# NOAA-GFDL/pace

Hardware: AMD Instinct MI355X
Metric: simulated-days/day + acoustic-step ms, C768 L79 fp64, 1/2/4/8 MI355X (higher is better)
Workload: dtype f64

## Files before the change

pace_amd/build.py:

```python
from __future__ import annotations

import argparse
import concurrent.futures as cf
import hashlib
import os
import subprocess
import sys

HERE = os.path.dirname(os.path.abspath(__file__))
CSRC = os.path.join(HERE, "csrc")
ROOT = os.path.dirname(HERE)
HOSTEMU_DIR = os.path.join(ROOT, "tests", "_hostemu")

SOURCES = ["fv3_ctx.hip", "fv3_tp2d.hip", "fv3_tp2x.hip", "fv3_tp4.hip", "fv3_tp4x.hip", "fv3_a2b.hip", "fv3_csw.hip", "fv3_dsw.hip", "fv3_wind.hip", "fv3_nh.hip", "fv3_del2x.hip", "fv3_pgf.hip", "fv3_step.hip", "fv3_halo.hip", "fv3_tracer.hip", "fv3_remap.hip", "fv3_c2l.hip", "fv3_diag.hip"]
HEADERS = ["fv3_common.h", "fv3_ops.h", "fv3_ppm.h", "fv3_a2b.h", "fv3_math.h", "fv3_agpr.h", "fv3_march.h", os.path.join("..", "..", "include", "fv3_mi355x.h")]

HIPCC = os.environ.get("HIPCC", "/opt/rocm/bin/hipcc")
HIP_FLAGS = ["--offload-arch=gfx950", "-std=c++17", "-O3", "-ffp-contract=off", "-fPIC", "-fno-gpu-rdc", "-Wno-unused-result"]
HOST_FLAGS = ["-x", "c++", "-std=c++17", "-O2", "-ffp-contract=off", "-fopenmp", "-fPIC", "-DFV3_HOST_EMU"]


def _tag() -> str:
    t = os.environ.get("FV3_LIB_TAG", "")
    return ("." + t) if t else ""


def lib_path(precision: int = 64, hostemu: bool = False) -> str:
    if hostemu:
        return os.path.join(HOSTEMU_DIR, f"libfv3_hostemu_f{precision}.so")
    return os.path.join(CSRC, f"libfv3_mi355x_f{precision}{_tag()}.so")


def _digest(paths, extra):
    h = hashlib.sha256()
    for p in paths:
        with open(p, "rb") as f:
            h.update(f.read())
    h.update(repr(extra).encode())
    return h.hexdigest()


def src_hash() -> str:
    paths = [os.path.join(CSRC, s) for s in SOURCES] + [os.path.normpath(os.path.join(CSRC, h)) for h in HEADERS]
    return _digest(paths, None)[:16]


def variant_suffix() -> str:
    extra = os.environ.get("FV3_EXTRA_FLAGS", "").split()
    per = sorted((k, v) for k, v in os.environ.items() if k.startswith("FV3_FLAGS_") and v.strip())
    tag = os.environ.get("FV3_LIB_TAG", "")
    if not extra and not per and not tag:
        return ""
    return "+" + hashlib.sha256(repr((extra, per)).encode()).hexdigest()[:8] + (("." + tag) if tag else "")


def _run(cmd):
    r = subprocess.run(cmd, capture_output=True, text=True)
    if r.returncode != 0:
        raise RuntimeError("build failed: " + " ".join(cmd) + "\n" + r.stdout + r.stderr)


def build(precision: int = 64, hostemu: bool = False, force: bool = False, verbose: bool = True) -> str:
    out = lib_path(precision, hostemu)
    objdir = os.path.join(HOSTEMU_DIR if hostemu else CSRC, f"_obj_f{precision}{'' if hostemu else _tag()}")
    os.makedirs(objdir, exist_ok=True)
    srcs = [os.path.join(CSRC, s) for s in SOURCES]
    hdrs = [os.path.normpath(os.path.join(CSRC, h)) for h in HEADERS]
    real = [] if precision == 64 else ["-DFV3_REAL=float"]
# ... 48 lines not shown
```

pace_amd/csrc/fv3_a2b.h:

```cpp
#pragma once
#include "fv3_ops.h"

#define A2B_A1 ((Real)0.5625)
#define A2B_A2 ((Real)-0.0625)
#define A2B_B1 ((Real)(7.0 / 12.0))
#define A2B_B2 ((Real)(-1.0 / 12.0))
#define A2B_C1 ((Real)(2.0 / 3.0))
#define A2B_C2 ((Real)(-1.0 / 6.0))
#define A2B_R3 ((Real)(1.0 / 3.0))

namespace {

struct A2B {
  const Geo &g;
  const Real *q;
  MPtr dxa;
  MPtr dya;
  bool W, E, S, N;

  Real sc;
  FV3_HD Real Q(int i, int j) const { return sc * q[IX(i, j)]; }

  FV3_HD Real qx_int(int i, int j) const { return A2B_B2 * (Q(i - 2, j) + Q(i + 1, j)) + A2B_B1 * (Q(i - 1, j) + Q(i, j)); }
  FV3_HD Real qy_int(int i, int j) const { return A2B_B2 * (Q(i, j - 2) + Q(i, j + 1)) + A2B_B1 * (Q(i, j - 1) + Q(i, j)); }

  FV3_HD Real qx_w1(int j) const {
    const Real g_in = dxa[IX(2, j)] / dxa[IX(1, j)], g_ou = dxa[IX(-1, j)] / dxa[IX(0, j)];
    return (Real)0.5 * ((((Real)2 + g_in) * Q(1, j) - Q(2, j)) / ((Real)1 + g_in) + (((Real)2 + g_ou) * Q(0, j) - Q(-1, j)) / ((Real)1 + g_ou));
  }
  FV3_HD Real qx_e1(int j) const {
    const int npx = g.npx;
    const Real g_in = dxa[IX(npx - 2, j)] / dxa[IX(npx - 1, j)], g_ou = dxa[IX(npx + 1, j)] / dxa[IX(npx, j)];
    return (Real)0.5 *
           ((((Real)2 + g_in) * Q(npx - 1, j) - Q(npx - 2, j)) / ((Real)1 + g_in) + (((Real)2 + g_ou) * Q(npx, j) - Q(npx + 1, j)) / ((Real)1 + g_ou));
  }
  FV3_HD Real qx(int i, int j) const {
    const int npx = g.npx;
    if (W) {
      if (i == 1) return qx_w1(j);
      if (i == 2) {
        const Real g_in = dxa[IX(2, j)] / dxa[IX(1, j)];
        return ((Real)3 * (g_in * Q(1, j) + Q(2, j)) - (g_in * qx_w1(j) + qx_int(3, j))) / ((Real)2 + (Real)2 * g_in);
      }
    }
    if (E) {
      if (i == npx) return qx_e1(j);
      if (i == npx - 1) {
        const Real g_in = dxa[IX(npx - 2, j)] / dxa[IX(npx - 1, j)];
        return ((Real)3 * (Q(npx - 2, j) + g_in * Q(npx - 1, j)) - (g_in * qx_e1(j) + qx_int(npx - 2, j))) / ((Real)2 + (Real)2 * g_in);
      }
    }
    return qx_int(i, j);
  }
  FV3_HD Real qy_s1(int i) const {
    const Real g_in = dya[IX(i, 2)] / dya[IX(i, 1)], g_ou = dya[IX(i, -1)] / dya[IX(i, 0)];
    return (Real)0.5 * ((((Real)2 + g_in) * Q(i, 1) - Q(i, 2)) / ((Real)1 + g_in) + (((Real)2 + g_ou) * Q(i, 0) - Q(i, -1)) / ((Real)1 + g_ou));
  }
  FV3_HD Real qy_n1(int i) const {
    const int npy = g.npy;
    const Real g_in = dya[IX(i, npy - 2)] / dya[IX(i, npy - 1)], g_ou = dya[IX(i, npy + 1)] / dya[IX(i, npy)];
    return (Real)0.5 *
           ((((Real)2 + g_in) * Q(i, npy - 1) - Q(i, npy - 2)) / ((Real)1 + g_in) + (((Real)2 + g_ou) * Q(i, npy) - Q(i, npy + 1)) / ((Real)1 + g_ou));
  }
  FV3_HD Real qy(int i, int j) const {
    const int npy = g.npy;
    if (S) {
      if (j == 1) return qy_s1(i);
      if (j == 2) {
        const Real g_in = dya[IX(i, 2)] / dya[IX(i, 1)];
        return ((Real)3 * (g_in * Q(i, 1) + Q(i, 2)) - (g_in * qy_s1(i) + qy_int(i, 3))) / ((Real)2 + (Real)2 * g_in);
      }
    }
    if (N) {
      if (j == npy) return qy_n1(i);
      if (j == npy - 1) {
        const Real g_in = dya[IX(i, npy - 2)] / dya[IX(i, npy - 1)];
        return ((Real)3 * (Q(i, npy - 2) + g_in * Q(i, npy - 1)) - (g_in * qy_n1(i) + qy_int(i, npy - 2))) / ((Real)2 + (Real)2 * g_in);
      }
    }
    return qy_int(i, j);
  }
  FV3_HD Real q2x(int ie_, int j) const {
    return (Q(ie_ - 1, j) * dxa[IX(ie_, j)] + Q(ie_, j) * dxa[IX(ie_ - 1, j)]) / (dxa[IX(ie_ - 1, j)] + dxa[IX(ie_, j)]);
  }
  FV3_HD Real q1y(int i, int je_) const {
    return (Q(i, je_ - 1) * dya[IX(i, je_)] + Q(i, je_) * dya[IX(i, je_ - 1)]) / (dya[IX(i, je_ - 1)] + dya[IX(i, je_)]);
  }
  FV3_HD Real edge_x(int ie_, int j, Real w) const { return w * q2x(ie_, j - 1) + ((Real)1 - w) * q2x(ie_, j); }
  FV3_HD Real edge_y(int i, int je_, Real w) const { return w * q1y(i - 1, je_) + ((Real)1 - w) * q1y(i, je_); }
  FV3_HD Real qxx_int(int i, int j) const { return A2B_A2 * (qx(i, j - 2) + qx(i, j + 1)) + A2B_A1 * (qx(i, j - 1) + qx(i, j)); }
  FV3_HD Real qyy_int(int i, int j) const { return A2B_A2 * (qy(i - 2, j) + qy(i + 1, j)) + A2B_A1 * (qy(i - 1, j) + qy(i, j)); }
};

FV3_HD inline Real extrap(Real fac, Real q1, Real q2) { return q1 + fac * (q1 - q2); }

FV3_HD inline __attribute__((always_inline)) Real a2b_point(const Geo &g, const Real *qlev, int t, int i, int j, Real scale = (Real)1) {
  const int fl = g.flags[t];
  const A2B a{g, qlev, g.dxa + t * g.st2, g.dya + t * g.st2, (fl & FV3_W) != 0, (fl & FV3_E) != 0, (fl & FV3_S) != 0, (fl & FV3_N) != 0, scale};
  const int npx = g.npx, npy = g.npy;
  const bool onW = a.W && i == 1, onE = a.E && i == npx, onS = a.S && j == 1, onN = a.N && j == npy;
  const Real *ce = g.corner_extrap + t * 12;
  Real r;
  if ((!a.W || i >= 3) && (!a.E || i <= npx - 2) && (!a.S || j >= 3) && (!a.N || j <= npy - 2)) {
    const Real *q = a.q;
    Real qx[4], qy[4];
#pragma unroll
    for (int n = 0; n < 4; ++n) {
      const int jj = j - 2 + n, ii = i - 2 + n;
      qx[n] = A2B_B2 * (scale * q[IX(i - 2, jj)] + scale * q[IX(i + 1, jj)]) + A2B_B1 * (scale * q[IX(i - 1, jj)] + scale * q[IX(i, jj)]);
      qy[n] = A2B_B2 * (scale * q[IX(ii, j - 2)] + scale * q[IX(ii, j + 1)]) + A2B_B1 * (scale * q[IX(ii, j - 1)] + scale * q[IX(ii, j)]);
    }
    const Real qxx = A2B_A2 * (qx[0] + qx[3]) + A2B_A1 * (qx[1] + qx[2]);
    const Real qyy = A2B_A2 * (qy[0] + qy[3]) + A2B_A1 * (qy[1] + qy[2]);
    r = (Real)0.5 * (qxx + qyy);
  } else if (onW && onS) {
    r = (extrap(ce[0], a.Q(1, 1), a.Q(2, 2)) + extrap(ce[1], a.Q(0, 1), a.Q(-1, 2)) + extrap(ce[2], a.Q(1, 0), a.Q(2, -1))) * A2B_R3;
  } else if (onE && onS) {
    r = (extrap(ce[3], a.Q(npx - 1, 1), a.Q(npx - 2, 2)) + extrap(ce[4], a.Q(npx - 1, 0), a.Q(npx - 2, -1)) + extrap(ce[5], a.Q(npx, 1), a.Q(npx + 1, 2))) *
        A2B_R3;
  } else if (onE && onN) {
    r = (extrap(ce[6], a.Q(npx - 1, npy - 1), a.Q(npx - 2, npy - 2)) + extrap(ce[7], a.Q(npx, npy - 1), a.Q(npx + 1, npy - 2)) +
         extrap(ce[8], a.Q(npx - 1, npy), a.Q(npx - 2, npy + 1))) *
        A2B_R3;
  } else if (onW && onN) {
    r = (extrap(ce[9], a.Q(1, npy - 1), a.Q(2, npy - 2)) + extrap(ce[10], a.Q(0, npy - 1), a.Q(-1, npy - 2)) + extrap(ce[11], a.Q(1, npy), a.Q(2, npy + 1))) *
        A2B_R3;
  } else if (onW) {
    r = a.edge_x(1, j, g.edge_w[t * g.nj + j + g.o]);
  } else if (onE) {
    r = a.edge_x(npx, j, g.edge_e[t * g.nj + j + g.o]);
  } else if (onS) {
    r = a.edge_y(i, 1, g.edge_s[t * g.ni + i + g.o]);
  } else if (onN) {
    r = a.edge_y(i, npy, g.edge_n[t * g.ni + i + g.o]);
  } else {
    Real qxx, qyy;
    if (a.S && j == 2)
      qxx = A2B_C1 * (a.qx(i, 1) + a.qx(i, 2)) + A2B_C2 * (a.edge_y(i, 1, g.edge_s[t * g.ni + i + g.o]) + a.qxx_int(i, 3));
    else if (a.N && j == npy - 1)
      qxx = A2B_C1 * (a.qx(i, npy - 2) + a.qx(i, npy - 1)) + A2B_C2 * (a.edge_y(i, npy, g.edge_n[t * g.ni + i + g.o]) + a.qxx_int(i, npy - 2));
    else
      qxx = a.qxx_int(i, j);
    if (a.W && i == 2)
      qyy = A2B_C1 * (a.qy(1, j) + a.qy(2, j)) + A2B_C2 * (a.edge_x(1, j, g.edge_w[t * g.nj + j + g.o]) + a.qyy_int(3, j));
    else if (a.E && i == npx - 1)
      qyy = A2B_C1 * (a.qy(npx - 2, j) + a.qy(npx - 1, j)) + A2B_C2 * (a.edge_x(npx, j, g.edge_e[t * g.nj + j + g.o]) + a.qyy_int(npx - 2, j));
    else
      qyy = a.qyy_int(i, j);
    r = (Real)0.5 * (qxx + qyy);
  }
  return r;
}

}

#define AB_OUT 61
#define AB_PF 4

struct A2bStore {
  Real *out;
  long st, sk;
  FV3_HD void operator()(int t, int k, unsigned p, Real v) const { (out + t * st + k * sk)[p] = v; }
};
template <int WPE, class Epi>
static void a2b_ord4_t(fv3_ctx *c, fv3_stream_t s, const Real *qin, int kin0, int kout0, int nk, Real scale, Epi epi) {
  const Geo g = c->g;
  const int kshift = kout0 - kin0;
  const Geo *gp = c->g_dev;
  const int nx = g.nx, ny = g.ny, nh = g.nh, npx = g.npx, npy = g.npy, sj32 = g.sj32, go = g.o;
  const long st = g.st, sk = g.sk;
  const int nstrip = (nx + 1 + AB_OUT - 1) / AB_OUT;
  const int seg = fv3_pick_seg((long)nstrip * ((ny + 64) / 64) * g.nsub * nk, 8);
  int nseg = (ny + 1 + seg / 2) / seg;
  if (nseg < 1) nseg = 1;
  const int seglen = (ny + 1 + nseg - 1) / nseg;
  const size_t smem = sizeof(Real) * 2 * (FV3_WAVE + 3);
  launch_waves<WPE>(c, s, nstrip, nseg, g.nsub * nk, smem, [=] FV3_HD(const Blk &blk, char *smem_) {
    const int t = blk.bz / nk, k = kin0 + (blk.bz - t * nk);
    const int fl = gp->flags[t];
    const Real *q = qin + t * st + k * sk;
    const int ia = (fl & FV3_W) ? 3 : 1, ib = (fl & FV3_E) ? npx - 2 : nx + 1;
    const int ja = (fl & FV3_S) ? 3 : 1, jb = (fl & FV3_N) ? npy - 2 : ny + 1;
    const int i0 = 1 + blk.bx * AB_OUT;
    int j0 = 1 + blk.by * seglen, j1 = j0 + seglen - 1;
    if (j0 < ja) j0 = ja;
    if (j1 > jb) j1 = jb;
    if (j0 > j1) return;
    const int ilo = i0 > ia ? i0 : ia, ihi = i0 + AB_OUT - 1 < ib ? i0 + AB_OUT - 1 : ib;
    if (ilo > ihi) return;
    Real *lq = (Real *)smem_ + 2;
    Real *ly = lq + FV3_WAVE + 3;
    const int ied = nx + nh;
    Real qa[FV3_LPT], qb[FV3_LPT], qc[FV3_LPT], qd[FV3_LPT];
    Real x0[FV3_LPT], x1[FV3_LPT], x2[FV3_LPT], x3[FV3_LPT];
    Real pf[AB_PF][FV3_LPT];
    unsigned pcol[FV3_LPT];
    bool own[FV3_LPT];
    const int r_beg = j0 - 2, r_end = j1 + 1;
    FV3_LANES(blk, lane, l) {
      const int i = i0 - 2 + lane, ic = i < ied ? i : ied;
      pcol[l] = (unsigned)(go * sj32 + ic + go);
      own[l] = i >= ilo && i <= ihi;
      qa[l] = qb[l] = qc[l] = qd[l] = x0[l] = x1[l] = x2[l] = x3[l] = (Real)0;
      if (lane < 2) lq[lane - 2] = ly[lane - 2] = (Real)0;
      if (lane == 0) lq[FV3_WAVE] = ly[FV3_WAVE] = (Real)0;
// ... 57 lines not shown
```

pace_amd/csrc/fv3_dsw.hip:

```cpp
#include "fv3_a2b.h"
#include "fv3_ops.h"
#include "fv3_ppm.h"

namespace {

struct FxAdv {
  Geo g;
  const Real *uc, *vc;
  long m2;
  Real dt;
  bool W, E, S, N;

  FV3_HD Real UC(int i, int j) const { return uc[IX(i, j)]; }
  FV3_HD Real VC(int i, int j) const { return vc[IX(i, j)]; }
  FV3_HD Real ut_gen(int i, int j) const {
    return (UC(i, j) - (Real)0.25 * (g.cosa_u + m2)[IX(i, j)] * (VC(i - 1, j) + VC(i, j) + VC(i - 1, j + 1) + VC(i, j + 1))) * (g.rsin_u + m2)[IX(i, j)];
  }
  FV3_HD Real vt_gen(int i, int j) const {
    return (VC(i, j) - (Real)0.25 * (g.cosa_v + m2)[IX(i, j)] * (UC(i, j - 1) + UC(i + 1, j - 1) + UC(i, j) + UC(i + 1, j))) * (g.rsin_v + m2)[IX(i, j)];
  }
  FV3_HD bool edge_col(int i) const { return (W && i == 1) || (E && i == g.npx); }
  FV3_HD bool edge_row(int j) const { return (S && j == 1) || (N && j == g.npy); }
  FV3_HD bool ut_special_row(int j) const { return (S && (j == 0 || j == 1)) || (N && (j == g.npy - 1 || j == g.npy)); }
  FV3_HD Real ut_edge(int i, int j) const {
// ... 775 lines not shown
  } else {
    for (int w = 0; w < wins.n; ++w) {
      Wins one, pone;
      one.n = pone.n = 1;
      one.w[0] = wins.w[w];
      pone.w[0] = patches.w[w];
      run(one, pone, &needs[w]);
    }
  }
}

bool dsw_honors_acc_first(const fv3_ctx *c) {
  int nmax = 0;
  for (int k = 0; k < c->g.nz; ++k) nmax = std::max(nmax, std::max(c->nord_v_h[k], std::max(c->nord_w_h[k], c->nord_t_h[k])));
  const char *sc_env = getenv("FV3_DSW_SCALARS");
  return !(sc_env && !strcmp(sc_env, "separate")) && nmax <= 2 && c->zeros;
}

struct AccSlots {
  const Real *crx[FV3_ACC_MAXSTEPS], *cry[FV3_ACC_MAXSTEPS];
};
static int acc_sum(fv3_ctx *c, Real *cx, Real *cy, int n, void *stream) {
  if (n < 1 || n > FV3_ACC_MAXSTEPS || (int)c->acc_slots.size() < 2 * n) return fv3_fail(c, FV3_ERR_ARG, "acc_sum: no Courant-number slots for this many sub-steps");
  AccSlots sl;
  for (int q = 0; q < FV3_ACC_MAXSTEPS; ++q) {
    const int m = q < n ? q : n - 1;
    sl.crx[q] = c->acc_slots[2 * m];
    sl.cry[q] = c->acc_slots[2 * m + 1];
  }
  const Geo g = c->g;
  const int isd = 1 - g.nh, ied = g.nx + g.nh, jsd = 1 - g.nh, jed = g.ny + g.nh;
  launch3<4>(c, (fv3_stream_t)stream, Box{isd, ied, jsd, jed, 0, g.nz - 1}, [=] FV3_HD(int t, int k, int i, int j) {
    const long p = t * g.st + k * g.sk + IX(i, j);
    if (i >= 1 && i <= g.nx + 1) {
      Real a = (Real)0 + sl.crx[0][p];
#pragma unroll
      for (int q = 1; q < FV3_ACC_MAXSTEPS; ++q)
        if (q < n) a = a + sl.crx[q][p];
      cx[p] = a;
    }
    if (j >= 1 && j <= g.ny + 1) {
      Real a = (Real)0 + sl.cry[0][p];
#pragma unroll
      for (int q = 1; q < FV3_ACC_MAXSTEPS; ++q)
        if (q < n) a = a + sl.cry[q][p];
      cy[p] = a;
    }
  });
  return fv3_post(c, (fv3_stream_t)stream, "acc_sum");
}

bool dsw_can_defer_acc(const fv3_ctx *c) { return dsw_honors_acc_first(c); }

int fv3_d_sw_out(fv3_ctx *c, const fv3_field *delpc_, const fv3_field *delp_, const fv3_field *pt_, const fv3_field *u_, const fv3_field *v_,
                 const fv3_field *w_, const fv3_field *uc_, const fv3_field *vc_, const fv3_field *ua_, const fv3_field *va_,
                 const fv3_field *divgd_, const fv3_field *mfx_, const fv3_field *mfy_, const fv3_field *cx_, const fv3_field *cy_,
                 const fv3_field *crx_, const fv3_field *cry_, const fv3_field *xfx_, const fv3_field *yfx_, const fv3_field *q_con_,
                 const fv3_field *zh_, const fv3_field *heat_source_, const fv3_field *diss_est_, double dtd, void *stream,
                 const fv3_field *o_delp_, const fv3_field *o_pt_, const fv3_field *o_w_, const fv3_field *o_q_con_, int (*after_scalars)(void *), void *after_user) {
  if (!c) return FV3_ERR_ARG;
  FV3_FIELD(delpc, delpc_) FV3_FIELD(delp, delp_) FV3_FIELD(pt, pt_) FV3_FIELD(u, u_) FV3_FIELD(v, v_) FV3_FIELD(w, w_) FV3_FIELD(uc, uc_)
  FV3_FIELD(vc, vc_) FV3_FIELD(ua, ua_) FV3_FIELD(va, va_) FV3_FIELD(divgd, divgd_) FV3_FIELD(mfx, mfx_) FV3_FIELD(mfy, mfy_) FV3_FIELD(cx, cx_)
  FV3_FIELD(cy, cy_) FV3_FIELD(crx, crx_) FV3_FIELD(cry, cry_) FV3_FIELD(xfx, xfx_) FV3_FIELD(yfx, yfx_) FV3_FIELD(q_con, q_con_)
  FV3_FIELD(heat_source, heat_source_)
  (void)zh_;
  (void)diss_est_;
  const bool oop = o_delp_ != nullptr;
  Real *o_delp = delp, *o_pt = pt, *o_w = w, *o_q_con = q_con;
  if (oop) {
    if (!o_pt_ || !o_w_ || !o_q_con_) return fv3_fail(c, FV3_ERR_ARG, "d_sw: the four output fields come together");
    o_delp = fv3_chk(c, o_delp_, "o_delp");
    o_pt = fv3_chk(c, o_pt_, "o_pt");
    o_w = fv3_chk(c, o_w_, "o_w");
    o_q_con = fv3_chk(c, o_q_con_, "o_q_con");
    if (!o_delp || !o_pt || !o_w || !o_q_con) return FV3_ERR_ARG;
    if (o_delp == delp || o_pt == pt || o_w == w || o_q_con == q_con) return fv3_fail(c, FV3_ERR_ARG, "d_sw: an output field aliases its input");
  }
  const Geo g = c->g;
  fv3_stream_t s = (fv3_stream_t)stream;
  const Real dt = (Real)dtd;
  const fv3_acoustic_config cf = c->cfg;
  const DampTables tab = c->tab;
  const int nz1 = g.nz - 1;
  const int isd = 1 - g.nh, ied = g.nx + g.nh, jsd = 1 - g.nh, jed = g.ny + g.nh;
  Real *ut = c->scratch[SC_A], *vt = c->scratch[SC_B], *fx = c->scratch[SC_C], *fy = c->scratch[SC_D], *gx = c->scratch[SC_E], *gy = c->scratch[SC_F];
  Real *heat_s = c->scratch[SC_H], *ke = c->scratch[SC_I], *wk = c->scratch[SC_J];
  int nord_max_v = 0, nord_max_w = 0, nord_max_t = 0, nord_max = 0;
  for (int k = 0; k < g.nz; ++k) {
    nord_max_v = std::max(nord_max_v, c->nord_v_h[k]);
    nord_max_w = std::max(nord_max_w, c->nord_w_h[k]);
    nord_max_t = std::max(nord_max_t, c->nord_t_h[k]);
    nord_max = std::max(nord_max, c->nord_h[k]);
  }

  fv3_stream_t s2 = fv3_aux(c, s);
  Real *dA_x = c->scratch[SC_DN_FX], *dA_y = c->scratch[SC_DN_FY], *dB_x = c->scratch[SC_S], *dB_y = c->scratch[SC_T], *d2w = c->scratch[SC_DN_D2];
  Deln dn_vt{g.nord_v, tab.tp_vt, g.damp_vt, 0, (Real)0, false, (Real)1.0e-4, nord_max_v};
  Deln dn_w{g.nord_w, tab.d6_w, g.damp_w, 0, (Real)0, false, (Real)1.0e-5, nord_max_w};
  Deln dn_t{g.nord_t, tab.tp_t, g.damp_t, 0, (Real)0, false, (Real)1.0e-4, nord_max_t};
  const char *sc_env = getenv("FV3_DSW_SCALARS");
  const bool fused_scalars = !(sc_env && !strcmp(sc_env, "separate")) && nord_max_v <= 2 && nord_max_t <= 2 && nord_max_w <= 2;
  if (c->seq_acc_first && !fused_scalars) return fv3_fail(c, FV3_ERR_ARG, "d_sw: the sequencer's first-sub-step form of the accumulators needs the fused scalar marches");
  const int scalars_mode = sc_env && !strcmp(sc_env, "quad") ? 0 : 1;
  const bool acc_defer = c->seq_acc_defer;
  if (acc_defer && !fused_scalars) return fv3_fail(c, FV3_ERR_ARG, "d_sw: the sequencer's deferred accumulation needs the fused scalar marches (fxadv with the Courant numbers)");
  if (fused_scalars) {
// ... 294 lines not shown
    const Real vd = damp * d;
    (vdamp + b)[p] = vd;
    (ke + b)[p] += vd;
  });
  Real *dnew = divgd;
  {
    if (!dd_sep) {
      divdamp_staged(c, s, divgd, uc, vc, nord_max, 0, nz1, nullptr);
    } else if (nord_max > 0) {
      dnew = c->scratch[SC_L];
      if (ks1 >= 0) divdamp_stream(c, ss, divgd, dnew, uc, vc, c->scratch[SC_M], nord_max, 0, ks1);
    }
  }
  {
    const Real dddmp = (Real)cf.dddmp;
    const bool keep_divgd = !(c->seq_divgd_dead && dd_sep);
    if (ks1 >= 0) a2b_ord4_t<8>(c, ss, wk, 0, 0, ks1 + 1, (Real)1, [=] FV3_HD(int t, int k, unsigned p, Real wkbv) {
      const int nord = g.nord[k];
      if (nord == 0) return;
      const long b = t * g.st + k * g.sk;
      const Real dpc = dd_sep ? (divgd + b)[p] : (delpc + b)[p];
      Real vo = (Real)0;
      if (dddmp >= (Real)1.0e-5) vo = fabs(dt) * sqrt(dpc * dpc + wkbv * wkbv);
      const Real damp2 = g.da_min_c * fv3_max(g.d2_divg[k], fv3_min((Real)0.20, dddmp * vo));
      const Real dn_ = (dnew + b)[p];
      if (keep_divgd) (divgd + b)[p] = dn_;
      const Real vd = damp2 * dpc + tab.dd8[k] * dn_;
      (vdamp + b)[p] = vd;
      (ke + b)[p] += vd;
    });
    if (ss != s) fv3_signal(c, ss, 4);
    if (kfz <= nz1) {
      Real *const wuc = c->scratch[SC_TP_FY2], *const wvc = c->scratch[SC_TP_FX2];
      dd_copy_windows(c, s, uc, vc, wuc, wvc, kfz, nz1, 2);
      divdamp_patches(c, s, divgd, dnew, wuc, wvc, c->scratch[SC_M], nord_max, kfz, nz1);
      WindStage ws{u, v, uc, vc, divgd, ke, vdamp, wk, dnew, tab.dd8, dt, dddmp, cf.hord_mt, keep_divgd, kfz, nz1};
      const char *sd = getenv("FV3_DSW_SIDE");
      if (heat_in_march && s == s_main && !(sd && !strcmp(sd, "copy"))) {
        ws.u_side = c->scratch[SC_N];
        ws.v_side = c->scratch[SC_O];
        ws.side_seg = sx_march_seg(c, nz1 - fdw_k0 + 1);
        side_from = kfz;
      }
      if (getenv("FV3_DEBUG_FD")) fprintf(stderr, "[d_sw] side copies by the wind stage: %s (segment %d)\n", ws.u_side ? "yes" : "no", ws.side_seg);
      wind_stage_march(c, s, ws);
      launch_frame_w(c, s, Frame{{Box{1, 3, 1, g.ny + 1, kfz, nz1}, Box{g.npx - 2, g.npx, 1, g.ny + 1, 0, 0}, Box{1, g.nx + 1, 1, 3, 0, 0}, Box{1, g.nx + 1, g.npy - 2, g.npy, 0, 0}}},
                     [=] FV3_HD(int w_, int t, int k, int i, int j) {
        const int fl = g.flags[t];
        if (!(fl & (w_ == 0 ? FV3_W : w_ == 1 ? FV3_E : w_ == 2 ? FV3_S : FV3_N))) return;
        if (w_ >= 2 && (((fl & FV3_W) && i <= 3) || ((fl & FV3_E) && i >= g.npx - 2))) return;
        ke_point(t, k, i, j);
      });
      const int nfr = g.nx + 1 > g.ny + 1 ? g.nx + 1 : g.ny + 1;
      launch3(c, s, Box{1, nfr, 1, 12, kfz, nz1}, [=] FV3_HD(int t, int k, int a_, int side) {
        const int fl = g.flags[t];
        int i, j;
        if (side <= 6) {
          if (a_ > g.ny + 1) return;
          if (!(fl & (side <= 3 ? FV3_W : FV3_E))) return;
          i = side <= 3 ? side : g.npx - 6 + side;
          j = a_;
        } else {
          if (a_ > g.nx + 1) return;
          if (!(fl & (side <= 9 ? FV3_S : FV3_N))) return;
          j = side <= 9 ? side - 6 : g.npy - 12 + side;
          i = a_;
          if (((fl & FV3_W) && i <= 3) || ((fl & FV3_E) && i >= g.npx - 2)) return;
        }
        const long b = t * g.st + k * g.sk;
        const unsigned p = IX(i, j);
        const Real wkbv = a2b_point(g, wk + b, t, i, j);
        const Real dpc = (divgd + b)[p];
        Real vo = (Real)0;
        if (dddmp >= (Real)1.0e-5) vo = fabs(dt) * sqrt(dpc * dpc + wkbv * wkbv);
        const Real damp2 = g.da_min_c * fv3_max(g.d2_divg[k], fv3_min((Real)0.20, dddmp * vo));
        const Real vd = damp2 * dpc + tab.dd8[k] * (dnew + b)[p];
        (vdamp + b)[p] = vd;
        (ke + b)[p] += vd;
      });
      dd_copy_windows(c, s, wuc, wvc, uc, vc, kfz, nz1, 0);
      if (keep_divgd) launch3(c, s, Box{1, g.nx + 1, 1, g.ny + 1, kfz, nz1}, [=] FV3_HD(int t, int k, int i, int j) {
        const long pp = t * g.st + k * g.sk + IX(i, j);
        divgd[pp] = dnew[pp];
      });
    }
  }

  };
  static const bool wind_overlap_off = !(getenv("FV3_DSW_WIND_OVERLAP") && getenv("FV3_DSW_WIND_OVERLAP")[0] == '1');
  for (int k = 0; k < g.nz; ++k) keep_uv_dx = keep_uv_dx || (c->d_con_h[k] > 1.0e-5 && !(c->damp_vt_h[k] > 1.0e-5));
  const bool wind_overlap = fused_scalars && s2 != s && !wind_overlap_off && !keep_uv_dx;
  if (wind_overlap) {
    fv3_wait(c, s2, 5);
    wind_branch(s2);
    fv3_signal(c, s2, 6);
  }

  if (after_scalars) {
    const int hst = after_scalars(after_user);
    if (hst != FV3_OK) return hst;
  }
  if (wind_overlap)
    fv3_wait(c, s, 6);
  else
    wind_branch(s);
  if (sponge_forked) fv3_wait(c, s, 4);

// ... 75 lines not shown
```

pace_amd/csrc/fv3_pgf.hip:

```cpp
#include "fv3_a2b.h"
#include "fv3_math.h"

#ifndef PG_WPE
#define PG_WPE (sizeof(Real) == 4 ? 3 : 2)
#endif

namespace {

#define PG_OUT 60
#define PG_PF 2
#define PG_NF 7
#ifndef PG_KB
#define PG_KB 16
#endif

struct PgfArgs {
  const Real *pp, *pk3, *gz, *delp;
  Real *u, *v;
  Real dt, top, gz_scale;
  int nz;
};

struct PgfCorner {
  Real g0, g1, k0, k1, q0, q1, w;
};

FV3_HD inline void pgf_update(const Geo &g, const PgfArgs &a, int t, int k, int i, int j, unsigned p, const PgfCorner &c, const PgfCorner &e, const PgfCorner &n, Real rx,
                              Real ry) {
  const long b = t * g.st + k * g.sk;
  const Real wkp = c.k1 - c.k0;
  if (i <= g.nx) {
    const Real du = a.dt / (wkp + (e.k1 - e.k0)) * ((c.g1 - e.g0) * (e.k1 - c.k0) + (c.g0 - e.g1) * (c.k1 - e.k0));
    (a.u + b)[p] = ((a.u + b)[p] + du + a.dt / (c.w + e.w) * ((c.g1 - e.g0) * (e.q1 - c.q0) + (c.g0 - e.g1) * (c.q1 - e.q0))) * rx;
  }
  if (j <= g.ny) {
    const Real dv = a.dt / (wkp + (n.k1 - n.k0)) * ((c.g1 - n.g0) * (n.k1 - c.k0) + (c.g0 - n.g1) * (c.k1 - n.k0));
    (a.v + b)[p] = ((a.v + b)[p] + dv + a.dt / (c.w + n.w) * ((c.g1 - n.g0) * (n.q1 - c.q0) + (c.g0 - n.g1) * (c.q1 - n.q0))) * ry;
  }
}

FV3_HD inline void pgf_march_range(const Geo &g, int fl, int &ia, int &ib, int &ja, int &jb) {
  ia = (fl & FV3_W) ? 3 : 1;
  ib = (fl & FV3_E) ? g.npx - 3 : g.nx + 1;
  ja = (fl & FV3_S) ? 3 : 1;
  jb = (fl & FV3_N) ? g.npy - 3 : g.ny + 1;
}

}

void nh_pgf_fused(fv3_ctx *c, fv3_stream_t s, const Real *pp, const Real *pk3, const Real *gz, const Real *delp, Real *u, Real *v, Real dt, Real top, Real gz_scale,
                  int pass) {
  const Geo g = c->g;
  const PgfArgs a{pp, pk3, gz, delp, u, v, dt, top, gz_scale, g.nz};
  const int nz = g.nz;
  const int F = FV3_FRAME_W;
  const bool has_frame = (g.nx + 1 > 2 * F) && (g.ny + 1 > 2 * F);
  const MPtr rdx = g.rdx, rdy = g.rdy;
  Real *ppb = c->scratch[SC_B], *pk3b = c->scratch[SC_C], *gzb = c->scratch[SC_D], *wk1 = c->scratch[SC_A];
  const int nxp = g.nx + 1, nyp = g.ny + 1;
  auto winds_at = [=] FV3_HD(int t, int k, int i, int j) {
    const long b = t * g.st + k * g.sk, b1 = b + g.sk;
    const unsigned p = IX(i, j), pe_ = IX(i + 1, j), pn = IX(i, j + 1);
    const PgfCorner cc{(gzb + b)[p], (gzb + b1)[p], (pk3b + b)[p], (pk3b + b1)[p], (ppb + b)[p], (ppb + b1)[p], (wk1 + b)[p]};
    PgfCorner ce = cc, cn = cc;
    if (i <= g.nx) ce = PgfCorner{(gzb + b)[pe_], (gzb + b1)[pe_], (pk3b + b)[pe_], (pk3b + b1)[pe_], (ppb + b)[pe_], (ppb + b1)[pe_], (wk1 + b)[pe_]};
    if (j <= g.ny) cn = PgfCorner{(gzb + b)[pn], (gzb + b1)[pn], (pk3b + b)[pn], (pk3b + b1)[pn], (ppb + b)[pn], (ppb + b1)[pn], (wk1 + b)[pn]};
    pgf_update(g, a, t, k, i, j, p, cc, ce, cn, (rdx + t * g.st2)[p], (rdy + t * g.st2)[p]);
  };
  const bool edges_now = pass != 2;
  if (edges_now) {
    const int nfr = nxp > nyp ? nxp : nyp;
    auto sides = [=](const Real *qin, Real *out, int k0, int k1, Real scale) {
      launch3(c, s, Box{1, nfr, 1, 8, k0, k1}, [=] FV3_HD(int t, int k, int a_, int side) {
        const int fl = g.flags[t];
        int i, j;
        if (side <= 4) {
          if (a_ > nyp) return;
          if (!(fl & (side <= 2 ? FV3_W : FV3_E))) return;
          i = side <= 2 ? side : g.npx - 4 + side;
          j = a_;
        } else {
          if (a_ > nxp) return;
          if (!(fl & (side <= 6 ? FV3_S : FV3_N))) return;
          j = side <= 6 ? side - 4 : g.npy - 8 + side;
          i = a_;
          if (((fl & FV3_W) && i <= 2) || ((fl & FV3_E) && i >= g.npx - 1)) return;
        }
        const long b = t * g.st + k * g.sk;
        (out + b)[IX(i, j)] = a2b_point(g, qin + b, t, i, j, scale);
      });
    };
    sides(a.gz, gzb, 0, nz, a.gz_scale);
    sides(a.pk3, pk3b, 1, nz, (Real)1);
    sides(a.pp, ppb, 1, nz, (Real)1);
    sides(a.delp, wk1, 0, nz - 1, (Real)1);
    launch_frame(c, s, Frame{{Box{1, 3, 1, nyp, 0, 0}, Box{g.npx - 2, g.npx, 1, nyp, 0, 0}, Box{4, g.npx - 3, 1, 3, 0, 0}, Box{4, g.npx - 3, g.npy - 2, g.npy, 0, 0}}},
                 [=] FV3_HD(int t, int, int i, int j) {
      const long p = t * g.st + IX(i, j);
      pk3b[p] = a.top;
      ppb[p] = (Real)0;
    });
  }
  const int nx = g.nx, ny = g.ny, nh = g.nh, sj32 = g.sj32, go = g.o;
  const long st = g.st, sk = g.sk, st2 = g.st2;
  const Geo *gp = c->g_dev;
  const int nstrip = (nx + 1 + PG_OUT - 1) / PG_OUT;
  const int seg = fv3_pick_seg((long)nstrip * ((ny + 64) / 64) * g.nsub * nz, 2);
  auto march = [&](const int sel, const int jlo, const int jhi) {
  if (jlo > jhi) return;
  const int nrow = jhi - jlo + 1;
  int nseg = (nrow + seg / 2) / seg;
  if (nseg < 1) nseg = 1;
  const int seglen = (nrow + nseg - 1) / nseg;
  const bool exports = edges_now;
  const int nblk = (nz + PG_KB - 1) / PG_KB;
  launch_waves<PG_WPE>(c, s, PG_KB, nstrip * nseg, g.nsub * nblk, 0, [=] FV3_HD(const Blk &blk_, char *) {
    const int t = blk_.bz / nblk, k = (blk_.bz - t * nblk) * PG_KB + blk_.bx;
    if (k >= nz) return;
    Blk blk = blk_;
    blk.by = blk_.by / nstrip;
    blk.bx = blk_.by - blk.by * nstrip;
    const int fl = gp->flags[t];
    const long b = t * st + k * sk, m2 = t * st2;
    int ia, ib, ja, jb;
    pgf_march_range(*gp, fl, ia, ib, ja, jb);
    const int i0 = 1 + blk.bx * PG_OUT;
// ... 153 lines not shown
```

Before: 213.4.

## Stage west/east tile-edge a2b stencils through LDS tiles in pgf and d_sw

```diff
diff --git a/pace_amd/build.py b/pace_amd/build.py
--- a/pace_amd/build.py
+++ b/pace_amd/build.py
@@ -13,7 +13,7 @@
 HOSTEMU_DIR = os.path.join(ROOT, "tests", "_hostemu")
 
 SOURCES = ["fv3_ctx.hip", "fv3_tp2d.hip", "fv3_tp2x.hip", "fv3_tp4.hip", "fv3_tp4x.hip", "fv3_a2b.hip", "fv3_csw.hip", "fv3_dsw.hip", "fv3_wind.hip", "fv3_nh.hip", "fv3_del2x.hip", "fv3_pgf.hip", "fv3_step.hip", "fv3_halo.hip", "fv3_tracer.hip", "fv3_remap.hip", "fv3_c2l.hip", "fv3_diag.hip"]
-HEADERS = ["fv3_common.h", "fv3_ops.h", "fv3_ppm.h", "fv3_a2b.h", "fv3_math.h", "fv3_agpr.h", "fv3_march.h", os.path.join("..", "..", "include", "fv3_mi355x.h")]
+HEADERS = ["fv3_common.h", "fv3_ops.h", "fv3_ppm.h", "fv3_a2b.h", "fv3_wetile.h", "fv3_math.h", "fv3_agpr.h", "fv3_march.h", os.path.join("..", "..", "include", "fv3_mi355x.h")]
 
 HIPCC = os.environ.get("HIPCC", "/opt/rocm/bin/hipcc")
 HIP_FLAGS = ["--offload-arch=gfx950", "-std=c++17", "-O3", "-ffp-contract=off", "-fPIC", "-fno-gpu-rdc", "-Wno-unused-result"]
diff --git a/pace_amd/csrc/fv3_a2b.h b/pace_amd/csrc/fv3_a2b.h
--- a/pace_amd/csrc/fv3_a2b.h
+++ b/pace_amd/csrc/fv3_a2b.h
@@ -1,5 +1,6 @@
 #pragma once
 #include "fv3_ops.h"
+#include "fv3_wetile.h"
 
 #define A2B_A1 ((Real)0.5625)
 #define A2B_A2 ((Real)-0.0625)
@@ -11,26 +12,34 @@
 
 namespace {
 
+template <class P>
+struct A2bPlane {
+  P p;
+  int o, sj32;
+  FV3_HD Real operator()(int i, int j) const { return p[(unsigned)((j + o) * sj32 + (i + o))]; }
+};
+
+template <class QA, class DA>
 struct A2B {
   const Geo &g;
-  const Real *q;
-  MPtr dxa;
+  QA q;
+  DA dxa;
   MPtr dya;
   bool W, E, S, N;
 
   Real sc;
-  FV3_HD Real Q(int i, int j) const { return sc * q[IX(i, j)]; }
+  FV3_HD Real Q(int i, int j) const { return sc * q(i, j); }
 
   FV3_HD Real qx_int(int i, int j) const { return A2B_B2 * (Q(i - 2, j) + Q(i + 1, j)) + A2B_B1 * (Q(i - 1, j) + Q(i, j)); }
   FV3_HD Real qy_int(int i, int j) const { return A2B_B2 * (Q(i, j - 2) + Q(i, j + 1)) + A2B_B1 * (Q(i, j - 1) + Q(i, j)); }
 
   FV3_HD Real qx_w1(int j) const {
-    const Real g_in = dxa[IX(2, j)] / dxa[IX(1, j)], g_ou = dxa[IX(-1, j)] / dxa[IX(0, j)];
+    const Real g_in = dxa(2, j) / dxa(1, j), g_ou = dxa(-1, j) / dxa(0, j);
     return (Real)0.5 * ((((Real)2 + g_in) * Q(1, j) - Q(2, j)) / ((Real)1 + g_in) + (((Real)2 + g_ou) * Q(0, j) - Q(-1, j)) / ((Real)1 + g_ou));
   }
   FV3_HD Real qx_e1(int j) const {
     const int npx = g.npx;
-    const Real g_in = dxa[IX(npx - 2, j)] / dxa[IX(npx - 1, j)], g_ou = dxa[IX(npx + 1, j)] / dxa[IX(npx, j)];
+    const Real g_in = dxa(npx - 2, j) / dxa(npx - 1, j), g_ou = dxa(npx + 1, j) / dxa(npx, j);
     return (Real)0.5 *
            ((((Real)2 + g_in) * Q(npx - 1, j) - Q(npx - 2, j)) / ((Real)1 + g_in) + (((Real)2 + g_ou) * Q(npx, j) - Q(npx + 1, j)) / ((Real)1 + g_ou));
   }
@@ -39,14 +48,14 @@
     if (W) {
       if (i == 1) return qx_w1(j);
       if (i == 2) {
-        const Real g_in = dxa[IX(2, j)] / dxa[IX(1, j)];
+        const Real g_in = dxa(2, j) / dxa(1, j);
         return ((Real)3 * (g_in * Q(1, j) + Q(2, j)) - (g_in * qx_w1(j) + qx_int(3, j))) / ((Real)2 + (Real)2 * g_in);
       }
     }
     if (E) {
       if (i == npx) return qx_e1(j);
       if (i == npx - 1) {
-        const Real g_in = dxa[IX(npx - 2, j)] / dxa[IX(npx - 1, j)];
+        const Real g_in = dxa(npx - 2, j) / dxa(npx - 1, j);
         return ((Real)3 * (Q(npx - 2, j) + g_in * Q(npx - 1, j)) - (g_in * qx_e1(j) + qx_int(npx - 2, j))) / ((Real)2 + (Real)2 * g_in);
       }
     }
@@ -81,7 +90,7 @@
     return qy_int(i, j);
   }
   FV3_HD Real q2x(int ie_, int j) const {
-    return (Q(ie_ - 1, j) * dxa[IX(ie_, j)] + Q(ie_, j) * dxa[IX(ie_ - 1, j)]) / (dxa[IX(ie_ - 1, j)] + dxa[IX(ie_, j)]);
+    return (Q(ie_ - 1, j) * dxa(ie_, j) + Q(ie_, j) * dxa(ie_ - 1, j)) / (dxa(ie_ - 1, j) + dxa(ie_, j));
   }
   FV3_HD Real q1y(int i, int je_) const {
     return (Q(i, je_ - 1) * dya[IX(i, je_)] + Q(i, je_) * dya[IX(i, je_ - 1)]) / (dya[IX(i, je_ - 1)] + dya[IX(i, je_)]);
@@ -94,21 +103,22 @@
 
 FV3_HD inline Real extrap(Real fac, Real q1, Real q2) { return q1 + fac * (q1 - q2); }
 
-FV3_HD inline __attribute__((always_inline)) Real a2b_point(const Geo &g, const Real *qlev, int t, int i, int j, Real scale = (Real)1) {
+template <class QA, class DA>
+FV3_HD inline __attribute__((always_inline)) Real a2b_point_acc(const Geo &g, const QA &qa, const DA &da, int t, int i, int j, Real scale) {
   const int fl = g.flags[t];
-  const A2B a{g, qlev, g.dxa + t * g.st2, g.dya + t * g.st2, (fl & FV3_W) != 0, (fl & FV3_E) != 0, (fl & FV3_S) != 0, (fl & FV3_N) != 0, scale};
+  const A2B<QA, DA> a{g, qa, da, g.dya + t * g.st2, (fl & FV3_W) != 0, (fl & FV3_E) != 0, (fl & FV3_S) != 0, (fl & FV3_N) != 0, scale};
   const int npx = g.npx, npy = g.npy;
   const bool onW = a.W && i == 1, onE = a.E && i == npx, onS = a.S && j == 1, onN = a.N && j == npy;
   const Real *ce = g.corner_extrap + t * 12;
   Real r;
   if ((!a.W || i >= 3) && (!a.E || i <= npx - 2) && (!a.S || j >= 3) && (!a.N || j <= npy - 2)) {
-    const Real *q = a.q;
+    const QA &q = a.q;
     Real qx[4], qy[4];
 #pragma unroll
     for (int n = 0; n < 4; ++n) {
       const int jj = j - 2 + n, ii = i - 2 + n;
-      qx[n] = A2B_B2 * (scale * q[IX(i - 2, jj)] + scale * q[IX(i + 1, jj)]) + A2B_B1 * (scale * q[IX(i - 1, jj)] + scale * q[IX(i, jj)]);
-      qy[n] = A2B_B2 * (scale * q[IX(ii, j - 2)] + scale * q[IX(ii, j + 1)]) + A2B_B1 * (scale * q[IX(ii, j - 1)] + scale * q[IX(ii, j)]);
+      qx[n] = A2B_B2 * (scale * q(i - 2, jj) + scale * q(i + 1, jj)) + A2B_B1 * (scale * q(i - 1, jj) + scale * q(i, jj));
+      qy[n] = A2B_B2 * (scale * q(ii, j - 2) + scale * q(ii, j + 1)) + A2B_B1 * (scale * q(ii, j - 1) + scale * q(ii, j));
     }
     const Real qxx = A2B_A2 * (qx[0] + qx[3]) + A2B_A1 * (qx[1] + qx[2]);
     const Real qyy = A2B_A2 * (qy[0] + qy[3]) + A2B_A1 * (qy[1] + qy[2]);
@@ -151,6 +161,21 @@
   }
   return r;
 }
+FV3_HD inline __attribute__((always_inline)) Real a2b_point(const Geo &g, const Real *qlev, int t, int i, int j, Real scale = (Real)1) {
+  return a2b_point_acc(g, A2bPlane<const Real *>{qlev, g.o, g.sj32}, A2bPlane<MPtr>{g.dxa + t * g.st2, g.o, g.sj32}, t, i, j, scale);
+}
+
+#ifndef FV3_HOST_EMU
+struct A2bTileAcc {
+  WeTile T;
+  int n;
+  FV3_HD Real operator()(int i, int j) const { return T.at(n, i, j); }
+};
+FV3_HD inline __attribute__((always_inline)) Real a2b_point_tile(const Geo &g, const WeTile &T, int t, int i, int j, Real scale = (Real)1) {
+  return a2b_point_acc(g, A2bTileAcc{T, 0}, A2bTileAcc{T, 1}, t, i, j, scale);
+}
+inline WeWin a2b_we_win(const Geo &g, int ncol) { return WeWin{1, ncol, -1, 4, g.npx - ncol + 1, g.npx, g.npx - 4, g.npx + 1, 1, g.ny + 1, 3, 2}; }
+#endif
 
 }
 
diff --git a/pace_amd/csrc/fv3_dsw.hip b/pace_amd/csrc/fv3_dsw.hip
--- a/pace_amd/csrc/fv3_dsw.hip
+++ b/pace_amd/csrc/fv3_dsw.hip
@@ -851,6 +851,43 @@
 
 bool dsw_can_defer_acc(const fv3_ctx *c) { return dsw_honors_acc_first(c); }
 
+struct WeDamp {
+  const Real *wk, *divgd, *dnew;
+  Real *vdamp, *ke;
+  const Real *dd8;
+  Real dt, dddmp;
+};
+static bool we_corner_tiled(const fv3_ctx *c) {
+#ifdef FV3_HOST_EMU
+  (void)c;
+  return false;
+#else
+  return fv3_we_tile_on() && fv3_we_fits(c->g, a2b_we_win(c->g, 3));
+#endif
+}
+static bool we_corner_damping(fv3_ctx *c, fv3_stream_t s, const WeDamp d, int k0, int k1) {
+#ifdef FV3_HOST_EMU
+  (void)s, (void)d, (void)k0, (void)k1;
+  return we_corner_tiled(c);
+#else
+  if (!we_corner_tiled(c)) return false;
+  const Geo g = c->g;
+  launch_we_tiles<2>(c, s, WeFields<2>{{d.wk, (const Real *)g.dxa}, {false, true}}, a2b_we_win(g, 3), k0, k1, [=] FV3_HD(const WeTile &T, int t, int k, int i, int j) {
+    const long b = t * g.st + k * g.sk;
+    const unsigned p = IX(i, j);
+    const Real wkbv = a2b_point_tile(g, T, t, i, j);
+    const Real dpc = (d.divgd + b)[p];
+    Real vo = (Real)0;
+    if (d.dddmp >= (Real)1.0e-5) vo = fabs(d.dt) * sqrt(dpc * dpc + wkbv * wkbv);
+    const Real damp2 = g.da_min_c * fv3_max(g.d2_divg[k], fv3_min((Real)0.20, d.dddmp * vo));
+    const Real vd = damp2 * dpc + d.dd8[k] * (d.dnew + b)[p];
+    (d.vdamp + b)[p] = vd;
+    (d.ke + b)[p] += vd;
+  });
+  return true;
+#endif
+}
+
 int fv3_d_sw_out(fv3_ctx *c, const fv3_field *delpc_, const fv3_field *delp_, const fv3_field *pt_, const fv3_field *u_, const fv3_field *v_,
                  const fv3_field *w_, const fv3_field *uc_, const fv3_field *vc_, const fv3_field *ua_, const fv3_field *va_,
                  const fv3_field *divgd_, const fv3_field *mfx_, const fv3_field *mfy_, const fv3_field *cx_, const fv3_field *cy_,
@@ -1251,7 +1288,9 @@
         ke_point(t, k, i, j);
       });
       const int nfr = g.nx + 1 > g.ny + 1 ? g.nx + 1 : g.ny + 1;
-      launch3(c, s, Box{1, nfr, 1, 12, kfz, nz1}, [=] FV3_HD(int t, int k, int a_, int side) {
+      const int side0 = we_corner_damping(c, s, WeDamp{wk, divgd, dnew, vdamp, ke, tab.dd8, dt, dddmp}, kfz, nz1) ? 7 : 1;
+      if (getenv("FV3_DEBUG_FD")) fprintf(stderr, "[d_sw] W / E tile-edge corner vorticity + damping: %s\n", side0 == 7 ? "LDS tiles" : "per-point launch");
+      launch3(c, s, Box{1, nfr, side0, 12, kfz, nz1}, [=] FV3_HD(int t, int k, int a_, int side) {
         const int fl = g.flags[t];
         int i, j;
         if (side <= 6) {
diff --git a/pace_amd/csrc/fv3_pgf.hip b/pace_amd/csrc/fv3_pgf.hip
--- a/pace_amd/csrc/fv3_pgf.hip
+++ b/pace_amd/csrc/fv3_pgf.hip
@@ -44,6 +44,29 @@
   ib = (fl & FV3_E) ? g.npx - 3 : g.nx + 1;
   ja = (fl & FV3_S) ? 3 : 1;
   jb = (fl & FV3_N) ? g.npy - 3 : g.ny + 1;
+}
+
+bool pgf_we_tiled(const fv3_ctx *c) {
+#ifdef FV3_HOST_EMU
+  (void)c;
+  return false;
+#else
+  return fv3_we_tile_on() && fv3_we_fits(c->g, a2b_we_win(c->g, 2));
+#endif
+}
+bool pgf_we_sides(fv3_ctx *c, fv3_stream_t s, const Real *qin, Real *out, int k0, int k1, Real scale) {
+#ifdef FV3_HOST_EMU
+  (void)c, (void)s, (void)qin, (void)out, (void)k0, (void)k1, (void)scale;
+  return false;
+#else
+  if (!pgf_we_tiled(c)) return false;
+  const Geo g = c->g;
+  const WeWin w = a2b_we_win(g, 2);
+  launch_we_tiles<2>(c, s, WeFields<2>{{qin, (const Real *)g.dxa}, {false, true}}, w, k0, k1, [=] FV3_HD(const WeTile &T, int t, int k, int i, int j) {
+    (out + t * g.st + k * g.sk)[IX(i, j)] = a2b_point_tile(g, T, t, i, j, scale);
+  });
+  return true;
+#endif
 }
 
 }
@@ -70,8 +93,10 @@
   const bool edges_now = pass != 2;
   if (edges_now) {
     const int nfr = nxp > nyp ? nxp : nyp;
+    if (getenv("FV3_DEBUG_FD")) fprintf(stderr, "[nh_p_grad] W / E tile-edge corners: %s\n", pgf_we_tiled(c) ? "LDS tiles" : "per-point launch");
     auto sides = [=](const Real *qin, Real *out, int k0, int k1, Real scale) {
-      launch3(c, s, Box{1, nfr, 1, 8, k0, k1}, [=] FV3_HD(int t, int k, int a_, int side) {
+      const int side0 = pgf_we_sides(c, s, qin, out, k0, k1, scale) ? 5 : 1;
+      launch3(c, s, Box{1, nfr, side0, 8, k0, k1}, [=] FV3_HD(int t, int k, int a_, int side) {
         const int fl = g.flags[t];
         int i, j;
         if (side <= 4) {
diff --git a/pace_amd/csrc/fv3_wetile.h b/pace_amd/csrc/fv3_wetile.h
--- /dev/null
+++ b/pace_amd/csrc/fv3_wetile.h
@@ -0,0 +1,102 @@
+#pragma once
+#include "fv3_common.h"
+
+inline bool fv3_we_tile_on() {
+#ifdef FV3_HOST_EMU
+  return false;
+#else
+  const char *e = getenv("FV3_WE_TILE");
+  return !(e && e[0] == '0');
+#endif
+}
+
+#ifndef FV3_HOST_EMU
+#define WE_COLS 16
+#define WE_RB 64
+#define WE_THREADS 256
+#define WE_HALO_MAX 8
+
+struct WeTile {
+  const Real *lds;
+  int pitch;
+  int c0, j0;
+  FV3_HD Real at(int n, int i, int j) const { return lds[(n * WE_COLS + (i - c0)) * pitch + (j - j0)]; }
+};
+
+inline int fv3_we_pitch(int rows) {
+  if (sizeof(Real) == 8) return rows | 1;
+  int p = rows;
+  while ((p & 31) != 2) ++p;
+  return p;
+}
+
+struct WeWin {
+  int iw0, iw1, nw0, nw1;
+  int ie0, ie1, ne0, ne1;
+  int j0, j1, hlo, hhi;
+};
+template <int NF>
+struct WeFields {
+  const Real *p[NF];
+  bool is2d[NF];
+};
+
+inline int fv3_we_col0(const Geo &g, int need_lo, int need_hi) {
+  int cs = (need_lo + g.o) & ~(WE_COLS - 1);
+  if (cs + WE_COLS - 1 < need_hi + g.o || cs + WE_COLS > g.ni) cs = std::min(need_lo + g.o, g.ni - WE_COLS);
+  return cs;
+}
+inline bool fv3_we_fits(const Geo &g, const WeWin &w) {
+  return g.ni >= WE_COLS && w.hlo >= 0 && w.hhi >= 0 && w.hlo + w.hhi <= WE_HALO_MAX && w.nw0 + g.o >= 0 && w.ne1 + g.o <= g.ni - 1 && w.nw1 - w.nw0 < WE_COLS && w.ne1 - w.ne0 < WE_COLS &&
+         (w.iw1 - w.iw0 + 1) * WE_RB <= WE_THREADS && (w.ie1 - w.ie0 + 1) * WE_RB <= WE_THREADS && w.iw0 >= w.nw0 && w.iw1 <= w.nw1 &&
+         w.ie0 >= w.ne0 && w.ie1 <= w.ne1;
+}
+
+template <int NF, class F>
+inline void launch_we_tiles(const fv3_ctx *c, fv3_stream_t s, const WeFields<NF> fs, const WeWin w, int k0, int k1, F f) {
+  const Geo &g = c->g;
+  const int nrows = w.j1 - w.j0 + 1, nk = k1 - k0 + 1;
+  if (nrows <= 0 || nk <= 0) return;
+  const int nrb = (nrows + WE_RB - 1) / WE_RB;
+  const int pitch = fv3_we_pitch(WE_RB + w.hlo + w.hhi);
+  const size_t smem = sizeof(Real) * NF * WE_COLS * pitch;
+  const int o = g.o, sj32 = g.sj32, nj = g.nj;
+  const long st = g.st, sk = g.sk, st2 = g.st2;
+  const int csw = fv3_we_col0(g, w.nw0, w.nw1), cse = fv3_we_col0(g, w.ne0, w.ne1);
+  const Geo *gp = c->g_dev;
+  launch_blocks(c, s, nrb, 2, g.nsub * nk, WE_THREADS, smem, [=] FV3_HD(const Blk &blk, char *smem_) {
+    const int t = blk.bz / nk, k = k0 + (blk.bz - t * nk), east = blk.by;
+    if (!(gp->flags[t] & (east ? FV3_E : FV3_W))) return;
+    Real *lds = (Real *)smem_;
+    const int jb0 = w.j0 + blk.bx * WE_RB, jb1 = jb0 + WE_RB - 1 < w.j1 ? jb0 + WE_RB - 1 : w.j1;
+    const int jt0 = jb0 - w.hlo, nr = jb1 - jb0 + 1 + w.hlo + w.hhi;
+    const int cs = east ? cse : csw;
+    constexpr int NIT = ((WE_RB + WE_HALO_MAX) * WE_COLS + WE_THREADS - 1) / WE_THREADS;
+    Real v[NF][NIT];
+#pragma unroll
+    for (int n = 0; n < NF; ++n) {
+      const Real *base = fs.is2d[n] ? fs.p[n] + t * st2 : fs.p[n] + t * st + k * sk;
+#pragma unroll
+      for (int it = 0; it < NIT; ++it) {
+        const int idx = blk.tid + it * WE_THREADS, r = idx / WE_COLS, cc = idx - r * WE_COLS;
+        int sr = jt0 + (r < nr ? r : nr - 1) + o;
+        sr = sr < 0 ? 0 : sr > nj - 1 ? nj - 1 : sr;
+        v[n][it] = FV3_EL(base, sr * sj32 + cs + cc);
+      }
+    }
+#pragma unroll
+    for (int n = 0; n < NF; ++n) {
+#pragma unroll
+      for (int it = 0; it < NIT; ++it) {
+        const int idx = blk.tid + it * WE_THREADS, r = idx / WE_COLS, cc = idx - r * WE_COLS;
+        if (r < nr) lds[(n * WE_COLS + cc) * pitch + r] = v[n][it];
+      }
+    }
+    blk.sync();
+    const WeTile T{lds, pitch, cs - o, jt0};
+    const int i0 = east ? w.ie0 : w.iw0, ncol = (east ? w.ie1 : w.iw1) - i0 + 1;
+    const int col = blk.tid / WE_RB, j = jb0 + (blk.tid - col * WE_RB);
+    if (col < ncol && j <= jb1) f(T, t, k, i0 + col, j);
+  });
+}
+#endif
```

New measurement: 214.3, median of 6. No clear change (+0.4%).
